# yanielc/medical-vision-textural-bias

Hardware: AMD Instinct MI355X
Metric: BraTS 4ch 240^3 vols/sec filtered+train-step @1/2/4/8 GPU; filter HBM GB/s (higher is better)
Workload: dtype f32

## Files before the change

### include/texbias.h

```cpp
#ifndef TEXBIAS_H
#define TEXBIAS_H

#include <stddef.h>
#include <stdint.h>

#ifdef __cplusplus
extern "C" {
#endif

#define TB_VERSION 1

#define TB_OK 0
#define TB_ERR_INVALID_ARG 1
#define TB_ERR_UNSUPPORTED_SIZE 2
#define TB_ERR_HIP 3
#define TB_ERR_WORKSPACE 4

#define TB_OP_NONE 0
#define TB_OP_DISK 1
#define TB_OP_GIBBS 2
#define TB_OP_LAYER 3
#define TB_OP_WRAP 4
#define TB_OP_SPIKE 5
#define TB_OP_ZF 6
// ... 104 lines not shown
int tb_channel_sum_ws_f32(const float* x, float* out, int64_t N, int64_t C, int64_t S, void* ws, size_t ws_bytes,
                          void* stream);

int tb_conv3d_small_f32(const float* x, const float* w, const float* b, float* y, int N, int Cin, int Cout, int D,
                        int H, int W, void* stream);
int tb_conv3d_small_add_f32(const float* x, const float* w, const float* b, const float* add, float* y, int N, int Cin,
                            int Cout, int D, int H, int W, void* stream);

int tb_conv3d_s2_fewin_f32(const float* in, const float* K, const float* bias, float* out, int N, int Cin, int Mout,
                           int Do, int Ho, int Wo, void* stream);
int tb_convT3d_fewout_f32(const float* x, const float* W, const float* bias, float* y, int N, int Cin, int Mout, int Di,
                          int Hi, int Wi, void* stream);
int tb_conv3d_fwd16_f32(const float* x, const float* W, const float* bias, float* y, int N, int D, int H, int Wd,
                        void* stream);
int tb_conv3d_fwd16_add_f32(const float* x, const float* W, const float* bias, const float* add, float* y, int N, int D,
                            int H, int Wd, void* stream);
int tb_conv3d_fwd16_dgrad_f32(const float* gy, const float* W, const float* add, int64_t add_sn, float* dx, int N, int D,
                              int H, int Wd, void* stream);

int tb_convT3d_mfma64_f32(const float* x, const float* W, const float* bias, float* y, int N, int Di, int Hi, int Wi,
                          void* stream);
int tb_convT3d_mfma_f32(const float* x, const float* W, const float* bias, float* y, int N, int Cin, int Di, int Hi,
                        int Wi, void* stream);

int tb_conv3d_mfma_f32(const float* x, const float* W, const float* bias, float* y, int N, int C, int D, int H, int Wd,
                       void* stream);
int tb_conv3d_mfma_add_f32(const float* x, const float* W, const float* bias, const float* add, float* y, int N, int C,
                           int D, int H, int Wd, void* stream);
int tb_conv3d_mfma_dgrad_f32(const float* gy, const float* W, const float* add, int64_t add_sn, float* dx, int N, int C,
                             int D, int H, int Wd, void* stream);

#define TB_CG_CONV 0
#define TB_CG_DGRAD 1
#define TB_CG_CONVT 2
size_t tb_conv3d_gemm_workspace_bytes(int mode, int N, int Cin, int M, int D, int H, int Wd, int stride, int ksize);
int tb_conv3d_gemm_f32(int mode, const float* x, int64_t xsn, const float* W, const float* bias, const float* add,
                       int64_t addsn, float* y, int64_t ysn, int N, int Cin, int M, int D, int H, int Wd, int stride,
                       int ksize, void* ws, size_t ws_bytes, void* stream);
int tb_conv3d_gemm_config(int mode, int N, int Cin, int M, int D, int H, int Wd, int stride, int ksize, int64_t* cfg);

size_t tb_conv3d_wgrad_gemm_ws_bytes(int N, int M, int C, int Do, int Ho, int Wo, int Di, int Hi, int Wi, int stride,
                                     int ksize);
int tb_conv3d_wgrad_gemm_f32(const float* G, int64_t gsn, const float* X, int64_t xsn, float* dW, int N, int M, int C,
                             int Do, int Ho, int Wo, int Di, int Hi, int Wi, int stride, int ksize, void* ws,
                             size_t ws_bytes, void* stream);
int tb_conv3d_wgrad_gemm_config(int N, int M, int C, int Do, int Ho, int Wo, int Di, int Hi, int Wi, int stride,
// ... 69 lines not shown
```

### medical-vision-textural-bias_amd/csrc/conv_up.hip

```cpp
#include <hip/hip_runtime.h>

#include <cstdlib>
#include <type_traits>

#include "conv_host.h"
#include "split_bf16.h"
#include "texbias.h"

namespace {

typedef float f2v __attribute__((ext_vector_type(2)));
typedef float f32x4 __attribute__((ext_vector_type(4)));
typedef const __attribute__((address_space(4))) float* cfloat_p;
typedef const __attribute__((address_space(4))) f2v* cf2v_p;

template <int B, int N, class F>
__device__ __forceinline__ void static_for(F&& f) {
  if constexpr (B < N) {
    f(std::integral_constant<int, B>{});
    static_for<B + 1, N>(f);
  }
}

struct S2Args {
// ... 811 lines not shown
#define TB_F16(X, PF)                                                                                             \
  case X:                                                                                                         \
    kern = add ? (NS == 4 ? k_conv3d_fwd16<YB, X, 512, true, PF, 4> : k_conv3d_fwd16<YB, X, 512, true, PF, 3>)     \
               : (NS == 4 ? k_conv3d_fwd16<YB, X, 512, false, PF, 4> : k_conv3d_fwd16<YB, X, 512, false, PF, 3>);  \
    break;
  switch (Wd / 16) {
    TB_F16(1, false) TB_F16(2, false) TB_F16(3, false) TB_F16(4, false) TB_F16(5, true) TB_F16(6, false)
    TB_F16(7, false) TB_F16(8, false)
    default: return TB_ERR_UNSUPPORTED_SIZE;
  }
#undef TB_F16
  a.ncol = N * a.nyb;
  unsigned nblk = (unsigned)(N * a.nyb * a.ZS);
  a.persist = per_cu == 1 && (int64_t)a.ncol * D >= 8LL * tb::num_cu() && nblk % tb::num_cu() != 0;
  if (a.persist) nblk = (unsigned)tb::num_cu();
  return tb::launch_lds(kern, dim3(nblk), dim3(512), lds, reinterpret_cast<hipStream_t>(stream), a);
}

namespace {
struct T64Args {
  const float* x;
  const float* W;
  const float* bias;
  float* y;
  int Di, Hi, Wi;
  int ZS, zlen, nyb;
  int PX, RX;
};

template <int G, int YB, int NL>
__global__ __launch_bounds__(256) void k_convT_mfma64(T64Args a) {
  extern __shared__ __attribute__((aligned(16))) float smem[];
  constexpr int NR = YB + 1;
  constexpr int CIN = 16 * G, HT = 4 / G;
  const int tid = (int)threadIdx.x, lane = tid & 63;
  const int w = __builtin_amdgcn_readfirstlane(tid >> 6);
  const int g = w % G, h = w / G;
  const int Di = a.Di, Hi = a.Hi, Wi = a.Wi, PX = a.PX, RX = a.RX, SS = CIN * RX;
  float* ring = smem;
  float* part = smem + 2 * SS;
  for (int i = tid; i < 2 * SS; i += 256) ring[i] = 0.f;
  int b = (int)blockIdx.x;
  const int zs = b % a.ZS;
  b /= a.ZS;
  const int yb = b % a.nyb, n = b / a.nyb;
  const int y0 = yb * YB;
  const int z0 = zs * a.zlen, z1 = min(Di, z0 + a.zlen);
  const int li = lane & 15, ks = lane >> 4;
  float af[108];
#pragma unroll
// ... 21 lines not shown
      const bool ok = in && gof[j] >= 0;
      rg[j] = *reinterpret_cast<const float4*>(src + gch[j] * cstride + (ok ? gof[j] : 0));
    }
  };
  auto store = [&](int zi) {
    float* d = ring + (zi & 1) * SS;
    const bool in = zi < Di;
#pragma unroll
    for (int j = 0; j < NL; ++j)
      *reinterpret_cast<float4*>(d + lof[j]) = (in && gof[j] >= 0) ? rg[j] : make_float4(0.f, 0.f, 0.f, 0.f);
  };
  float bm[4];
#pragma unroll
  for (int r = 0; r < 4; ++r) bm[r] = a.bias ? a.bias[4 * ks + r] : 0.f;
  __syncthreads();
  load(z0);
  store(z0);
  load(z0 + 1);
  store(z0 + 1);
  __builtin_amdgcn_s_waitcnt(0x0F70);
  __syncthreads();
  const int npos = YB * Wi, ntile = (npos + 15) / 16;
  const int64_t oplane = 4 * plane, orow = 2 * Wi;
  float* yb0 = a.y + (int64_t)n * 16 * (2 * Di) * oplane;
  auto sums = [&](int z, int t0, int pb) {
    const float* pr = part + pb * 4 * 8 * 256;
    for (int k = w; k < 4 * HT; k += 4) {
      const int hq = k >> 2, pz = (k >> 1) & 1, py = k & 1, q0 = pz * 4 + py * 2;
      const int pq = 16 * (t0 + hq) + li, yq = pq / Wi, xq = pq - yq * Wi;
      const bool okp = t0 + hq < ntile && pq < npos && y0 + yq < Hi;
#pragma unroll
      for (int r = 0; r < 4; ++r) {
        const int m = 4 * ks + r, e = m * 16 + li;
        float v0 = bm[r], v1 = bm[r];
#pragma unroll
        for (int v = 0; v < G; ++v) {
          v0 += pr[((hq * G + v) * 8 + q0) * 256 + e];
          v1 += pr[((hq * G + v) * 8 + q0 + 1) * 256 + e];
        }
        if (okp)
          *reinterpret_cast<float2*>(yb0 + ((int64_t)m * (2 * Di) + 2 * z + pz) * oplane +
                                     (int64_t)(2 * (y0 + yq) + py) * orow + 2 * xq) = make_float2(v0, v1);
      }
    }
  };
  int buf = 0;
  for (int z = z0; z < z1; ++z) {
    if (z + 1 < z1) load(z + 2);
    const float* sz[2] = {ring + (z & 1) * SS, ring + ((z + 1) & 1) * SS};
    for (int t0 = 0; t0 < ntile; t0 += HT) {
      const int tI = t0 + h;
      const int p = 16 * tI + li, pc = p < npos ? p : npos - 1;
      const int yy = pc / Wi, xx = pc - yy * Wi;
      const int bl = (16 * g + ks) * RX + yy * PX + xx;
      f32x4 acc[8];
#pragma unroll
      for (int q = 0; q < 8; ++q) acc[q] = f32x4{0.f, 0.f, 0.f, 0.f};
#pragma unroll
      for (int tz = 0; tz < 3; ++tz)
#pragma unroll
        for (int ty = 0; ty < 3; ++ty)
#pragma unroll
// ... 1 lines not shown
            const int t = tz * 9 + ty * 3 + tx;
            const int par = (tz != 1) * 4 + (ty != 1) * 2 + (tx != 1);
            const float* s = sz[tz == 0] + bl + (ty == 0) * PX + (tx == 0);
#pragma unroll
            for (int cq = 0; cq < 4; ++cq)
              acc[par] = __builtin_amdgcn_mfma_f32_16x16x4f32(af[4 * t + cq], s[4 * cq * RX], acc[par], 0, 0, 0);
          }
      float* pw = part + (buf * 4 + w) * 8 * 256;
#pragma unroll
      for (int q = 0; q < 8; ++q)
#pragma unroll
        for (int r = 0; r < 4; ++r) pw[q * 256 + (4 * ks + r) * 16 + li] = acc[q][r];
      __syncthreads();
      if (t0 > 0) sums(z, t0 - HT, buf ^ 1);
      buf ^= 1;
    }
    store(z + 2);
    sums(z, ((ntile - 1) / HT) * HT, buf ^ 1);
    __syncthreads();
  }
}
}

int tb_convT3d_mfma64_f32(const float* x, const float* W, const float* bias, float* y, int N, int Di, int Hi, int Wi,
                          void* stream) {
  return tb_convT3d_mfma_f32(x, W, bias, y, N, 64, Di, Hi, Wi, stream);
}

int tb_convT3d_mfma_f32(const float* x, const float* W, const float* bias, float* y, int N, int Cin, int Di, int Hi,
                        int Wi, void* stream) {
  if (!x || !W || !y || N < 1 || Di < 1 || Hi < 1 || Wi < 1) return TB_ERR_INVALID_ARG;
  if (Cin != 32 && Cin != 64) return TB_ERR_UNSUPPORTED_SIZE;
  if (Wi % 4 != 0 || Wi > 64 || (reinterpret_cast<uintptr_t>(x) & 15) != 0 || (reinterpret_cast<uintptr_t>(y) & 7) != 0)
    return TB_ERR_UNSUPPORTED_SIZE;
  constexpr int YB = 2;
  T64Args a{};
  a.x = x, a.W = W, a.bias = bias, a.y = y, a.Di = Di, a.Hi = Hi, a.Wi = Wi;
  a.PX = Wi + 4;
  a.RX = (YB + 1) * a.PX;
  while ((a.RX & 31) != 16) ++a.RX;
  a.nyb = (Hi + YB - 1) / YB;
  const size_t lds = (size_t)4 * (2 * Cin * a.RX + 2 * 4 * 8 * 256);
  if (lds > 163840) return TB_ERR_UNSUPPORTED_SIZE;
  a.zlen = tb::zseg(Di, N * a.nyb, 1, 1);
  a.ZS = (Di + a.zlen - 1) / a.zlen;
  const int nl = (Cin * (YB + 1) * (Wi / 4) + 255) / 256;
  void (*kern)(T64Args) = nullptr;
  switch (nl) {
#define TB_NL(k) \
  case k: kern = Cin == 64 ? k_convT_mfma64<4, YB, k> : k_convT_mfma64<2, YB, k>; break;
    TB_NL(1) TB_NL(2) TB_NL(3) TB_NL(4) TB_NL(5) TB_NL(6) TB_NL(7) TB_NL(8) TB_NL(9) TB_NL(10) TB_NL(11) TB_NL(12)
#undef TB_NL
    default: return TB_ERR_UNSUPPORTED_SIZE;
  }
  return tb::launch_lds(kern, dim3((unsigned)(N * a.nyb * a.ZS)), dim3(256), lds,
                        reinterpret_cast<hipStream_t>(stream), a);
}

namespace {
struct S1Args {
  const float* x;
  const float* W;
  const float* bias;
  const float* add;
  float* y;
  int D, H, Wd, YB;
  int ZS, zlen, nyb, MG;
  int PX, RX;
  int flip;
  int64_t addsn;
};

template <int G, int NC, int NL, int NTH, bool ADD = false>
__global__ __launch_bounds__(NTH) void k_conv3d_mfma_s1(S1Args a) {
  constexpr int CIN = 16 * G, MTB = 4 / G, NWG = NTH / 256;
  extern __shared__ __attribute__((aligned(16))) float smem[];
  const int tid = (int)threadIdx.x, lane = tid & 63;
  const int w = __builtin_amdgcn_readfirstlane(tid >> 6);
  const int g = w % G, mt = (w / G) % MTB, h = w / 4;
// ... 408 lines not shown
```

### medical-vision-textural-bias_amd/texbias/_lib.py

```python
from __future__ import annotations

import ctypes as C
import os
import threading

from ._abi import TB_OK

PKG_DIR = os.path.dirname(os.path.dirname(os.path.abspath(__file__)))
LIB_PATH = os.environ.get("TEXBIAS_LIB", os.path.join(PKG_DIR, "libtexbias.so"))

_lock = threading.Lock()
_lib = None


class TexbiasError(RuntimeError):
    pass


def _proto(L):
    P, I, I64, U64, F, SZ = C.c_void_p, C.c_int, C.c_int64, C.c_uint64, C.c_float, C.c_size_t
    sig = {
        "tb_version": (I, []),
        "tb_error_string": (C.c_char_p, [I]),
        "tb_last_hip_error": (I, []),
# ... 23 lines not shown
        "tb_conv3d_wgrad_bias_ws_f32": (I, [P, P, P, P] + [I] * 11 + [P, SZ, P, P]),
        "tb_instnorm_prelu_workspace_bytes": (SZ, [I64]),
        "tb_instnorm_prelu_fwd_f32": (I, [P, P, P, P, P, I64, I64, F, P, SZ, P]),
        "tb_instnorm_prelu_bwd_f32": (I, [P, P, P, P, P, P, P, I64, I64, P, SZ, P]),
        "tb_channel_sum_f32": (I, [P, P, I64, I64, I64, P]),
        "tb_channel_sum_ws_bytes": (SZ, [I64, I64, I64]),
        "tb_channel_sum_ws_f32": (I, [P, P, I64, I64, I64, P, SZ, P]),
        "tb_adn_workspace_bytes": (SZ, [I64, I64, I64]),
        "tb_adam_f32": (I, [I, P, P, P, P, P, P, P] + [C.c_double] * 5 + [I, P]),
        "tb_adn_counters": (I64, [I64, I64]),
        "tb_adn_fwd_f32": (I, [P, I64, P, I64, P, I64, P, P, P, I64, I64, I64, F, P, SZ, P, P]),
        "tb_adn_bwd_f32": (I, [P, I64, P, I64, P, I64, P, P, P, P, P, P, I64, I64, I64, P, SZ, P, P]),
        "tb_conv3d_small_f32": (I, [P, P, P, P] + [I] * 6 + [P]),
        "tb_conv3d_small_add_f32": (I, [P, P, P, P, P] + [I] * 6 + [P]),
        "tb_conv3d_fwd16_add_f32": (I, [P, P, P, P, P] + [I] * 4 + [P]),
        "tb_conv3d_mfma_add_f32": (I, [P, P, P, P, P] + [I] * 5 + [P]),
        "tb_conv3d_mfma_dgrad_f32": (I, [P, P, P, I64, P] + [I] * 5 + [P]),
        "tb_conv3d_fwd16_dgrad_f32": (I, [P, P, P, I64, P] + [I] * 4 + [P]),
        "tb_conv3d_s2_fewin_f32": (I, [P, P, P, P] + [I] * 6 + [P]),
        "tb_convT3d_fewout_f32": (I, [P, P, P, P] + [I] * 6 + [P]),
        "tb_conv3d_fwd16_f32": (I, [P, P, P, P] + [I] * 4 + [P]),
        "tb_convT3d_mfma64_f32": (I, [P, P, P, P] + [I] * 4 + [P]),
        "tb_convT3d_mfma_f32": (I, [P, P, P, P] + [I] * 5 + [P]),
        "tb_conv3d_mfma_f32": (I, [P, P, P, P] + [I] * 5 + [P]),
        "tb_conv3d_gemm_workspace_bytes": (SZ, [I] * 9),
        "tb_conv3d_gemm_f32": (I, [I, P, I64, P, P, P, I64, P, I64] + [I] * 8 + [P, SZ, P]),
        "tb_conv3d_gemm_config": (I, [I] * 9 + [P]),
        "tb_conv3d_wgrad_gemm_ws_bytes": (SZ, [I] * 11),
        "tb_conv3d_wgrad_gemm_f32": (I, [P, I64, P, I64, P] + [I] * 11 + [P, SZ, P]),
        "tb_conv3d_wgrad_gemm_config": (I, [I] * 11 + [P]),
        "tb_conv3d_wgrad_gemm_ws_bytes_ex": (SZ, [I] * 12),
        "tb_conv3d_wgrad_gemm_ex_f32": (I, [P, I64, P, I64, P] + [I] * 12 + [P, SZ, P]),
        "tb_conv3d_wgrad_gemm_config_ex": (I, [I] * 12 + [P]),
        "tb_dice_sums_f32": (I, [P, P, P, I64, I64, I, I, P]),
        "tb_dice_sums_ws_bytes": (SZ, [I64, I64]),
        "tb_dice_sums_ws_f32": (I, [P, P, P, I64, I64, I, I, P, SZ, P]),
        "tb_dice_sums_bwd_f32": (I, [P, P, P, P, I64, I64, I, I, P]),
        "tb_dice_metric_sums_f32": (I, [P, P, P, I64, I64, P]),
        "tb_dice_loss_f32": (I, [P, P, I64, I64, I, I, F, F, P]),
        "tb_dice_loss_bwd_f32": (I, [P, P, P, I64, I64, I, I, F, F, P]),
        "tb_set_compiled_plans": (I, [I]),
        "tb_set_chain_chunk": (I, [I]),
        "tb_set_pass_timing": (I, [I]),
        "tb_get_pass_times_ms": (I, [P, P]),
        "tb_get_pass_stats": (I, [P, P, P]),
        "tb_pass_kernel": (C.c_char_p, [I]),
# ... 38 lines not shown
```

### medical-vision-textural-bias_amd/texbias/conv.py

```python
from __future__ import annotations

import ctypes
import functools
import math
import os

import torch
import torch.nn as nn
import torch.nn.functional as F

from ._lib import TexbiasError, check, lib

MIN_K_PER_OUTPUT = 64
ENABLED = os.environ.get("TEXBIAS_WGRAD", "1") != "0"
CONVT64 = True
CONVMFMA = True
CONV16 = True


def _stream(t: torch.Tensor) -> int:
    return torch.cuda.current_stream(t.device).cuda_stream


@functools.lru_cache(maxsize=256)
# ... 174 lines not shown
        return False
    k, s, p = w.shape[2], stride[0], padding[0]
    if not ((k == 3 and p == 1 and s in (1, 2)) or (k == 1 and p == 0 and s == 1 and not transposed)):
        return False
    if transposed:
        if s != 2 or tuple(output_padding) != (1, 1, 1):
            return False
        g_shape = tuple(x.shape)
        x_shape = (x.shape[0], w.shape[1]) + tuple(2 * n for n in x.shape[2:])
    else:
        g_shape, x_shape = (x.shape[0], w.shape[0]) + tuple(out_spatial), tuple(x.shape)
    if not WGRAD_GEMM_MIN_POS <= math.prod(g_shape[2:]) <= WGRAD_GEMM_MAX_POS or \
            g_shape[1] * x_shape[1] < WGRAD_GEMM_MIN_MC:
        return False
    return _wgg_ws_bytes(g_shape[0], g_shape[1], x_shape[1], *g_shape[2:], *x_shape[2:], s, k, 0) > 0


GEMM = os.environ.get("TEXBIAS_CONVGEMM", "1") != "0"
GEMM_T = False
GEMM_1 = False
GEMM_TDX = False
FWD16_DX_ADD = True
MFMA_DX_ADD = False


def _gemm_geom_ok(x: torch.Tensor, w: torch.Tensor, stride, padding, transposed: bool, output_padding) -> bool:
    if not (GEMM and custom_backward_applies(x, w) and x.dim() == 5 and len(set(stride)) == 1 and
            len(set(padding)) == 1):
        return False
    k = tuple(w.shape[2:])
    s, p = stride[0], padding[0]
    if transposed:
        ok = k == (3, 3, 3) and s == 2 and p == 1 and tuple(output_padding) == (1, 1, 1) and x.shape[1] == w.shape[0]
    else:
        ok = x.shape[1] == w.shape[1] and ((k == (3, 3, 3) and p == 1 and s in (1, 2)) or
                                           (k == (1, 1, 1) and p == 0 and s == 1 and GEMM_1))
    return ok and x.shape[1] % 8 == 0 and x.numel() // x.shape[1] * 8 * max(w.shape[0], w.shape[1], x.shape[1]) < 2 ** 31


def gemm_applies(x, w, stride, padding, transposed: bool, output_padding=(0, 0, 0)) -> bool:
    return (GEMM_T or not transposed) and _gemm_geom_ok(x, w, stride, padding, transposed, output_padding)


def gemm_dgrad_applies(gy, x, w, stride, padding, transposed: bool, output_padding=(0, 0, 0)) -> bool:
    if not (_gemm_geom_ok(x, w, stride, padding, transposed, output_padding) and gy.is_cuda and
            gy.dtype == torch.float32):
# ... 66 lines not shown
                                          b.data_ptr() if b is not None else None, y.data_ptr(), N, Cin, Cout, D, H,
                                          W, _stream(x)), "tb_convT3d_fewout_f32")
    return y


def _s2_shape_ok(spatial) -> bool:
    D, H, W = spatial
    return D % 2 == 0 and H % 2 == 0 and W % 4 == 0 and W <= 160


def s2_fewin_applies(x: torch.Tensor, w: torch.Tensor, stride, padding) -> bool:
    return custom_backward_applies(x, w) and x.dim() == 5 and tuple(w.shape[2:]) == (3, 3, 3) and \
        x.shape[1] == w.shape[1] and tuple(stride) == (2, 2, 2) and tuple(padding) == (1, 1, 1) and w.shape[1] <= 4 and \
        w.shape[0] in (16, 32) and _s2_shape_ok(x.shape[2:]) and x.data_ptr() % 16 == 0


def convT_fewout_applies(x: torch.Tensor, w: torch.Tensor, stride, padding, output_padding) -> bool:
    return custom_backward_applies(x, w) and x.dim() == 5 and tuple(w.shape[2:]) == (3, 3, 3) and \
        x.shape[1] == w.shape[0] and tuple(stride) == (2, 2, 2) and tuple(padding) == (1, 1, 1) and \
        tuple(output_padding) == (1, 1, 1) and w.shape[1] <= 4 and w.shape[0] in (16, 32) and x.shape[-1] % 4 == 0 and x.shape[-1] <= 80 and \
        _s2_shape_ok(tuple(2 * n for n in x.shape[2:]))


def convT_mfma(x: torch.Tensor, w: torch.Tensor, b) -> torch.Tensor:
    x = x.contiguous()
    N, Cin, D, H, W = x.shape
    y = torch.empty((N, 16, 2 * D, 2 * H, 2 * W), dtype=torch.float32, device=x.device)
    with torch.cuda.device(x.device):
        check(lib().tb_convT3d_mfma_f32(x.data_ptr(), w.contiguous().data_ptr(),
                                        b.data_ptr() if b is not None else None, y.data_ptr(), N, Cin, D, H, W,
                                        _stream(x)), "tb_convT3d_mfma_f32")
    return y


convT_mfma64 = convT_mfma


def s2_dgrad_applies(gy: torch.Tensor, x: torch.Tensor, w: torch.Tensor, stride, padding) -> bool:
    return CONVT64 and gy.is_cuda and gy.dtype == torch.float32 and w.dtype == torch.float32 and \
        tuple(w.shape) == (32, 16, 3, 3, 3) and tuple(stride) == (2, 2, 2) and gy.shape[1] == 32 and \
        tuple(padding) == (1, 1, 1) and gy.dim() == 5 and all(2 * a == b for a, b in zip(gy.shape[2:], x.shape[2:])) and \
        gy.shape[-1] % 4 == 0 and gy.shape[-1] <= 64 and gy.data_ptr() % 16 == 0


def convT64_applies(x: torch.Tensor, w: torch.Tensor, stride, padding, output_padding) -> bool:
    return CONVT64 and custom_backward_applies(x, w) and x.dim() == 5 and tuple(w.shape) == (64, 16, 3, 3, 3) and \
        x.shape[1] == 64 and \
        tuple(stride) == (2, 2, 2) and tuple(padding) == (1, 1, 1) and tuple(output_padding) == (1, 1, 1) and \
        x.shape[-1] % 4 == 0 and x.shape[-1] <= 64 and x.data_ptr() % 16 == 0


def conv_fwd16(x: torch.Tensor, w: torch.Tensor, b, add=None) -> torch.Tensor:
    x = x.contiguous()
    N, _, D, H, W = x.shape
# ... 165 lines not shown
            if k == "small":
                return small_conv(x, w, b, add)
            return conv_gemm(x, w, b, "convT" if self.transposed else "conv", self.stride[0], self.k, add=add)
        if add is not None:
            return self.forward(x, w, b).add_(add)
        if k == "fwd16":
            return conv_fwd16(x, w, b)
        if k == "mfma":
            return conv_mfma(x, w, b)
        if k == "fewin":
            return conv_s2_fewin(x, s2_pairs(w), b, w.shape[0])
        if k == "small":
            return small_conv(x, w, b)
        if k == "fewout":
            return convT_fewout(x, w, b)
        if k == "convT64":
            return convT_mfma(x, w, b)
        if k == "gemm":
            return conv_gemm(x, w, b, "convT" if self.transposed else "conv", self.stride[0], self.k)
        if self.transposed:
            return F.conv_transpose3d(x, w, b, self.stride, self.padding, self.output_padding)
        return F.conv3d(x, w, b, self.stride, self.padding)

    def input_grad(self, gy, x, w, add=None):
        k = self.dx
        if add is not None:
            if k == "fwd16" and FWD16_DX_ADD:
                return conv_fwd16_dgrad(gy, w, add)
            if k == "mfma" and MFMA_DX_ADD:
                return conv_mfma_dgrad(gy, w, add)
            if k == "small":
                return small_conv(gy, w.flip(2, 3, 4).transpose(0, 1).contiguous(), None, add.contiguous())
            if k == "gemm" and not self.transposed and self.stride[0] == 1:
                return conv_gemm(gy, w, None, "dgrad", 1, w.shape[2], add=add.contiguous())
            return self.input_grad(gy, x, w).add_(add)
        if k == "fwd16":
            return conv_fwd16_dgrad(gy, w)
        if k == "mfma":
            return conv_mfma_dgrad(gy, w)
        if k == "small":
            return small_conv(gy, w.flip(2, 3, 4).transpose(0, 1).contiguous(), None)
        if k == "fewout":
            return conv_s2_fewin(gy, s2_pairs(w), None, w.shape[0])
        if k == "convT64":
            return convT_mfma(gy if gy.data_ptr() % 16 == 0 else gy.clone(), w, None)
        if k == "gemm":
            return gemm_dgrad(gy, w, self.stride[0], self.transposed)
        gx, _, _ = torch.ops.aten.convolution_backward(
            gy, x, w, None, list(self.stride), list(self.padding), [1, 1, 1], self.transposed,
            list(self.output_padding), 1, [True, False, False])
        return gx
# ... 72 lines not shown
```

### medical-vision-textural-bias_amd/texbias/unet.py

```python
from __future__ import annotations

import os
from typing import Sequence

import torch
import torch.nn as nn

from . import conv as _conv
from .conv import Conv3d, ConvTranspose3d
from . import norm as _norm
from .norm import adn_backward, adn_forward, instnorm_prelu

FUSED = os.environ.get("TEXBIAS_FUSED_UNITS", "1") != "0"


def _fusable(x: torch.Tensor, conv: nn.Module, adn) -> bool:
    if not (FUSED and _norm.ENABLED and x.is_cuda and x.dtype == torch.float32 and
            isinstance(conv, (Conv3d, ConvTranspose3d)) and conv.groups == 1 and conv.dilation == (1, 1, 1) and
            _conv.custom_backward_applies(x, conv.weight)):
        return False
    if isinstance(conv, Conv3d) and conv.padding_mode != "zeros":
        return False
    return adn is None or adn.D.p == 0.0 or not adn.training

# ... 41 lines not shown
        need_b = ctx.has_b and n[2]
        gb = None
        if n[1] and need_b:
            gw, gb = ctx.route.weight_bias_grad(g, x, w)
        else:
            gw = ctx.route.weight_grad(g, x, w) if n[1] else None
        if need_b and gb is None:
            gb = _conv.channel_sum(g)
        return gx, gw, gb, None


def _adjacent(a: torch.Tensor, b: torch.Tensor):
    if not (a.is_contiguous() and b.is_contiguous() and a.shape[1:] == b.shape[1:] and a.dtype == b.dtype and
            a.untyped_storage().data_ptr() == b.untyped_storage().data_ptr() and
            b.storage_offset() == a.storage_offset() + a.numel()):
        return None
    return torch.empty(0, dtype=a.dtype, device=a.device).set_(
        a.untyped_storage(), a.storage_offset(), (a.shape[0] + b.shape[0],) + tuple(a.shape[1:]))


class _StackedUnitFn(torch.autograd.Function):

    @staticmethod
    def forward(ctx, x, w0, b0, wr, br, a0w, w1, b1, a1w, unit, eps, skip):
        c = w0.shape[0]
        w_st = _adjacent(w0, wr)
        if w_st is None:
            w_st = torch.cat([w0, wr], 0)
        b_st = None
        if b0 is not None and br is not None:
            b_st = _adjacent(b0, br)
            if b_st is None:
                b_st = torch.cat([b0, br], 0)
        x = x.contiguous()
        r_st = unit.stacked_route(x, w_st)
        y2 = r_st.forward(x, w_st, b_st)
        z0, res = y2[:, :c], y2[:, c:]
        a0, m0, s0 = adn_forward(z0, a0w, eps)
        conv1 = list(unit.conv.children())[1].conv
        r1 = _conv.route_of(conv1, a0)
        z1 = r1.forward(a0, w1, b1)
        out, m1, s1 = adn_forward(z1, a1w, eps, res=res)
        ctx.save_for_backward(x, w_st, a0w, w1, a1w, y2, a0, z1, m0, s0, m1, s1)
        ctx.cfg = (c, r_st, r1, b0 is not None, b1 is not None)
        ctx.skip = skip
        return out

    @staticmethod
    def backward(ctx, g):
        x, w_st, a0w, w1, a1w, y2, a0, z1, m0, s0, m1, s1 = ctx.saved_tensors
        c, r_st, r1, has_b0, has_b1 = ctx.cfg
        n = ctx.needs_input_grad
        dy2 = torch.empty_like(y2)
        gs = ctx.skip.pop("g", None)
        if gs is not None:
            g = torch.add(g, gs, out=dy2[:, c:])
        else:
            g = g.contiguous()
            dy2[:, c:].copy_(g)
        dbr = torch.empty(c, dtype=g.dtype, device=g.device) if has_b0 and n[4] else None
        dz1, da1, db1 = adn_backward(z1, g, m1, s1, a1w, need_w=n[8], need_bias=has_b1, dysum_out=dbr)
        da0 = r1.input_grad(dz1, a0, w1)
        gw1 = r1.weight_grad(dz1, a0, w1) if n[6] else None
        _, dw0a, db0 = adn_backward(y2[:, :c], da0, m0, s0, a0w, need_w=n[5], need_bias=has_b0,
                                    dx_out=dy2[:, :c])
        gx = r_st.input_grad(dy2, x, w_st) if n[0] else None
        gw_st = r_st.weight_grad(dy2, x, w_st) if (n[1] or n[3]) else None
        return (gx, gw_st[:c] if gw_st is not None else None, db0, gw_st[c:] if gw_st is not None else None, dbr,
                dw0a, gw1, db1 if n[7] else None, da1, None, None, None)


class ADN(nn.Sequential):
    def __init__(self, channels: int, dropout: float = 0.0):
        super().__init__()
        self.add_module("N", nn.InstanceNorm3d(channels, eps=1e-5, affine=False, track_running_stats=False))
        self.add_module("D", nn.Dropout(p=dropout))
        self.add_module("A", nn.PReLU(num_parameters=1))

    def forward(self, x):
        if _norm.ENABLED and x.is_cuda and x.dtype == torch.float32 and (self.D.p == 0.0 or not self.training):
            return instnorm_prelu(x, self.A.weight, self.N.eps)
        return super().forward(x)


class Convolution(nn.Sequential):
    def __init__(self, cin: int, cout: int, strides: int = 1, kernel_size: int = 3, conv_only: bool = False,
                 is_transposed: bool = False, dropout: float = 0.0):
        super().__init__()
        pad = (kernel_size - 1) // 2
        if is_transposed:
            conv = ConvTranspose3d(cin, cout, kernel_size, stride=strides, padding=pad, output_padding=strides - 1)
        else:
# ... 33 lines not shown
            self.residual = nn.Identity()
        self._register_state_dict_hook(ResidualUnit._unshare_packed)

    @staticmethod
    def _unshare_packed(module, state_dict, prefix, local_metadata):
        for k in ("conv.unit0.conv.weight", "conv.unit0.conv.bias", "residual.weight", "residual.bias"):
            v = state_dict.get(prefix + k)
            if v is not None and not isinstance(v, nn.Parameter) and v.untyped_storage().nbytes() != \
                    v.numel() * v.element_size():
                state_dict[prefix + k] = v.clone()
        return state_dict

    def forward(self, x):
        units = list(self.conv.children())
        if isinstance(self.residual, Conv3d) and len(units) == 2 and all(hasattr(u, "adn") for u in units):
            u0, u1 = units
            r = self.residual
            if r.stride == u0.conv.stride and r.kernel_size == u0.conv.kernel_size and r.padding == u0.conv.padding \
                    and isinstance(u0.conv, Conv3d) and _fusable(x, u0.conv, u0.adn) and _fusable(x, r, None) and \
                    _fusable(x, u1.conv, u1.adn) and (r.bias is None) == (u0.conv.bias is None) and \
                    u0.adn.N.eps == u1.adn.N.eps and r.padding_mode == "zeros":
                skip = {}
                y = _StackedUnitFn.apply(x, u0.conv.weight, u0.conv.bias, r.weight, r.bias, u0.adn.A.weight,
                                         u1.conv.weight, u1.conv.bias, u1.adn.A.weight, self, u0.adn.N.eps, skip)
                y._tb_skip = skip
                return y
        if isinstance(self.residual, nn.Identity) and len(units) == 1 and hasattr(units[0], "adn"):
            out = self.__dict__.pop("_tb_out", None)
            if out is not None and tuple(out.shape) != tuple(x.shape[:1]) + (units[0].conv.out_channels,) + \
                    tuple(x.shape[2:]):
                out = None
            y = units[0].fused(x, res=x, out=out)
            if y is not None:
                return y
        if isinstance(self.residual, nn.Identity) and len(units) == 1 and not hasattr(units[0], "adn") and \
                _fusable(x, units[0].conv, None):
            c = units[0].conv
            return _ConvResFn.apply(x, c.weight, c.bias, _conv.route_of(c, x))
        res = self.residual(x)
        return self.conv(x) + res

    def pack_parameters(self) -> bool:
        units = list(self.conv.children())
        if not (isinstance(self.residual, Conv3d) and len(units) == 2 and hasattr(units[0], "conv")):
            return False
        c0, r = units[0].conv, self.residual
        if torch.is_inference_mode_enabled() or not isinstance(c0, Conv3d) or r.stride != c0.stride or \
# ... 122 lines not shown
```

Baseline: 197.4.

## Fuse skip-gradient add into transposed-conv dgrad and add split-bf16 convT kernel

Adds an add/strided-output variant of the transposed-conv MFMA kernel so the backward pass of a stacked residual unit can accumulate the upstream skip gradient and write directly into the concatenated dy2 buffer of the next unit. This is meant to remove a separate elementwise add and a copy into the concat buffer. It also adds a new 512-thread split-bf16 (3-way) MFMA kernel for Cin=64 with parity-class tap decomposition, plus a YB=1 fallback for larger widths. The cost is more complex autograd bookkeeping through shared skip dicts, and numerical differences from the bf16 split path.

After: 201.7, median of 6. +2.2%, better.

```diff
diff --git a/include/texbias.h b/include/texbias.h
--- a/include/texbias.h
+++ b/include/texbias.h
@@ -150,6 +150,8 @@
                           void* stream);
 int tb_convT3d_mfma_f32(const float* x, const float* W, const float* bias, float* y, int N, int Cin, int Di, int Hi,
                         int Wi, void* stream);
+int tb_convT3d_mfma_add_f32(const float* x, const float* W, const float* bias, const float* add, int64_t add_sn,
+                            float* y, int64_t y_sn, int N, int Cin, int Di, int Hi, int Wi, void* stream);
 
 int tb_conv3d_mfma_f32(const float* x, const float* W, const float* bias, float* y, int N, int C, int D, int H, int Wd,
                        void* stream);
diff --git a/medical-vision-textural-bias_amd/csrc/conv_up.hip b/medical-vision-textural-bias_amd/csrc/conv_up.hip
--- a/medical-vision-textural-bias_amd/csrc/conv_up.hip
+++ b/medical-vision-textural-bias_amd/csrc/conv_up.hip
@@ -857,10 +857,12 @@
   const float* x;
   const float* W;
   const float* bias;
+  const float* add;
   float* y;
   int Di, Hi, Wi;
   int ZS, zlen, nyb;
   int PX, RX;
+  int64_t ysn, addsn;
 };
 
 template <int G, int YB, int NL>
@@ -928,13 +930,22 @@
   __syncthreads();
   const int npos = YB * Wi, ntile = (npos + 15) / 16;
   const int64_t oplane = 4 * plane, orow = 2 * Wi;
-  float* yb0 = a.y + (int64_t)n * 16 * (2 * Di) * oplane;
+  float* yb0 = a.y + (int64_t)n * a.ysn;
+  const float* ab0 = a.add ? a.add + (int64_t)n * a.addsn : nullptr;
   auto sums = [&](int z, int t0, int pb) {
     const float* pr = part + pb * 4 * 8 * 256;
     for (int k = w; k < 4 * HT; k += 4) {
       const int hq = k >> 2, pz = (k >> 1) & 1, py = k & 1, q0 = pz * 4 + py * 2;
       const int pq = 16 * (t0 + hq) + li, yq = pq / Wi, xq = pq - yq * Wi;
       const bool okp = t0 + hq < ntile && pq < npos && y0 + yq < Hi;
+      float2 av[4];
+      if (ab0) {
+#pragma unroll
+        for (int r = 0; r < 4; ++r)
+          av[r] = okp ? *reinterpret_cast<const float2*>(ab0 + ((int64_t)(4 * ks + r) * (2 * Di) + 2 * z + pz) * oplane +
+                                                         (int64_t)(2 * (y0 + yq) + py) * orow + 2 * xq)
+                      : make_float2(0.f, 0.f);
+      }
 #pragma unroll
       for (int r = 0; r < 4; ++r) {
         const int m = 4 * ks + r, e = m * 16 + li;
@@ -944,6 +955,7 @@
           v0 += pr[((hq * G + v) * 8 + q0) * 256 + e];
           v1 += pr[((hq * G + v) * 8 + q0 + 1) * 256 + e];
         }
+        if (ab0) v0 += av[r].x, v1 += av[r].y;
         if (okp)
           *reinterpret_cast<float2*>(yb0 + ((int64_t)m * (2 * Di) + 2 * z + pz) * oplane +
                                      (int64_t)(2 * (y0 + yq) + py) * orow + 2 * xq) = make_float2(v0, v1);
@@ -991,39 +1003,286 @@
 }
 }
 
+namespace {
+struct TSArgs {
+  const float* x;
+  const float* W;
+  const float* bias;
+  const float* add;
+  float* y;
+  int Di, Hi, Wi, YB;
+  int ZS, zlen, nyb;
+  int ntile;
+  int64_t ysn, addsn;
+};
+
+struct CtTap {
+  int t, dz, dy, dx;
+};
+constexpr CtTap ct_tap(int cls, int j) {
+  const int pz = (cls >> 2) & 1, py = (cls >> 1) & 1, px = cls & 1;
+  const int nx = 1 + px, ny = 1 + py;
+  const int ix = j % nx, iy = (j / nx) % ny, iz = j / (nx * ny);
+  return CtTap{(pz ? (iz ? 0 : 2) : 1) * 9 + (py ? (iy ? 0 : 2) : 1) * 3 + (px ? (ix ? 0 : 2) : 1), pz ? iz : 0,
+               py ? iy : 0, px ? ix : 0};
+}
+constexpr int ct_ntap(int cls) { return (1 + ((cls >> 2) & 1)) * (1 + ((cls >> 1) & 1)) * (1 + (cls & 1)); }
+constexpr int ct_cls(int half, int s) {
+  return half == 0 ? (s < 4 ? 7 : s < 6 ? 3 : 0) : (s < 2 ? 5 : s < 4 ? 6 : s == 4 ? 1 : s == 5 ? 2 : 4);
+}
+constexpr int ct_pair(int half, int s) { return half == 0 ? (s < 4 ? s : s < 6 ? s - 4 : 0) : (s < 4 ? (s & 1) : 0); }
+constexpr CtTap ct_step_tap(int half, int s, int hi) {
+  const int cls = ct_cls(half, s), e = 2 * ct_pair(half, s) + hi;
+  return ct_tap(cls, e < ct_ntap(cls) ? e : ct_ntap(cls) - 1);
+}
+constexpr bool ct_step_pad(int half, int s, int hi) { return 2 * ct_pair(half, s) + hi >= ct_ntap(ct_cls(half, s)); }
+
+template <int HALF>
+__device__ __forceinline__ void ct_mma(const tb::bf16x8 (&af)[7][3], const char* rb, int sb0, int sb1, int RPB, int SPL,
+                                       int hv, char* pw) {
+  using tb::bf16x8;
+  bf16x8 bq[2][3];
+  auto ldb = [&](int s, bf16x8 (&bf)[3]) {
+    const CtTap t0 = ct_step_tap(HALF, s, 0), t1 = ct_step_tap(HALF, s, 1);
+    const int c0 = (t0.dz ? sb1 : sb0) + t0.dy * RPB + t0.dx * 32;
+    const int c1 = (t1.dz ? sb1 : sb0) + t1.dy * RPB + t1.dx * 32;
+    const int o = hv ? c1 : c0;
+    bf[1] = *reinterpret_cast<const bf16x8*>(rb + o + SPL);
+    bf[2] = *reinterpret_cast<const bf16x8*>(rb + o + 2 * SPL);
+    bf[0] = *reinterpret_cast<const bf16x8*>(rb + o);
+  };
+  tb::f32x4s c = {0.f, 0.f, 0.f, 0.f}, cs = c;
+  ldb(0, bq[0]);
+#pragma unroll
+  for (int s = 0; s < 7; ++s) {
+    if (s + 1 < 7) ldb(s + 1, bq[(s + 1) & 1]);
+    tb::mfma_split6(af[s], bq[s & 1], c, cs);
+    if (s == 6 || ct_cls(HALF, s + 1) != ct_cls(HALF, s)) {
+      c += cs;
+      *reinterpret_cast<tb::f32x4s*>(pw + ct_cls(HALF, s) * 1024) = c;
+      c = tb::f32x4s{0.f, 0.f, 0.f, 0.f}, cs = c;
+    }
+  }
+  __builtin_amdgcn_sched_group_barrier(0x100, 3, 0);
+#pragma unroll
+  for (int s = 0; s < 6; ++s) {
+    __builtin_amdgcn_sched_group_barrier(0x100, 3, 0);
+    __builtin_amdgcn_sched_group_barrier(0x008, 6, 0);
+  }
+  __builtin_amdgcn_sched_group_barrier(0x008, 6, 0);
+}
+
+template <bool ADD>
+__global__ __launch_bounds__(512) void k_convT_split(TSArgs a) {
+  using tb::bf16x8;
+  constexpr int G = 4, NTH = 512;
+  extern __shared__ __attribute__((aligned(16))) char ringt[];
+  const int tid = (int)threadIdx.x, lane = tid & 63;
+  const int w = __builtin_amdgcn_readfirstlane(tid >> 6);
+  const int grp = w & 3, half = w >> 2;
+  const int Di = a.Di, Hi = a.Hi, Wi = a.Wi, YB = a.YB, NR = YB + 1;
+  const int RPB = (Wi + 1) * 32, GPB = NR * RPB, SPL = G * GPB, SLOT = 3 * SPL;
+  char* part = ringt + 2 * SLOT;
+  for (int i = tid; i < 2 * SLOT / 16; i += NTH) reinterpret_cast<uint4*>(ringt)[i] = make_uint4(0, 0, 0, 0);
+  int b = (int)blockIdx.x;
+  const int zs = b % a.ZS;
+  b /= a.ZS;
+  const int yb = b % a.nyb, n = b / a.nyb;
+  const int y0 = yb * YB;
+  const int z0 = zs * a.zlen, z1 = min(Di, z0 + a.zlen);
+  const int li = lane & 15, g4 = lane >> 4, hi = g4 >> 1;
+  bf16x8 af[7][3];
+  {
+    const float* wl = a.W + ((16 * grp + 8 * (g4 & 1)) * 16 + li) * 27;
+#pragma unroll
+    for (int s = 0; s < 7; ++s) {
+      const int t = half ? (hi ? ct_step_tap(1, s, 1).t : ct_step_tap(1, s, 0).t)
+                         : (hi ? ct_step_tap(0, s, 1).t : ct_step_tap(0, s, 0).t);
+      const bool pad = hi && (half ? ct_step_pad(1, s, 1) : ct_step_pad(0, s, 1));
+      float v[8];
+#pragma unroll
+      for (int j = 0; j < 8; ++j) v[j] = wl[j * 16 * 27 + t];
+#pragma unroll
+      for (int j = 0; j < 8; ++j) v[j] = pad ? 0.f : v[j];
+      tb::split3(v, af[s][0], af[s][1], af[s][2]);
+    }
+  }
+  const int64_t plane = (int64_t)Hi * Wi, cstride = (int64_t)Di * plane;
+  const char* xb = reinterpret_cast<const char*>(a.x + (int64_t)n * 16 * G * cstride);
+  const int W4 = Wi >> 2, ntask = 4 * NR * W4 * G;
+  const int tk = tid < ntask ? tid : tid % ntask;
+  const int cq = tk & 3, rr = (tk >> 2) % NR, r2 = (tk >> 2) / NR, q4 = r2 % W4, sg = r2 / W4;
+  const int lof = sg * GPB + rr * RPB + 4 * q4 * 32 + cq * 8;
+  const int yi = y0 + rr;
+  const bool rowok = yi < Hi;
+  const unsigned chb = (unsigned)(4 * cstride);
+  const unsigned gof = rowok ? (unsigned)(16 * sg + 4 * cq) * chb + 4u * (unsigned)(yi * Wi + 4 * q4) : 0u;
+  float4 rg[4];
+  auto load = [&](int zi) {
+    const char* src = xb + (int64_t)(zi >= Di ? Di - 1 : zi) * plane * 4;
+#pragma unroll
+    for (int c = 0; c < 4; ++c) rg[c] = *reinterpret_cast<const float4*>(src + c * chb + gof);
+  };
+  auto store = [&](int zi) {
+    char* d = ringt + (zi & 1) * SLOT + lof;
+    const unsigned m = 0u - (unsigned)(rowok && zi < Di);
+#pragma unroll
+    for (int e = 0; e < 4; ++e) {
+      float v[4];
+#pragma unroll
+      for (int c = 0; c < 4; ++c)
+        v[c] = __uint_as_float(__float_as_uint(e == 0 ? rg[c].x : e == 1 ? rg[c].y : e == 2 ? rg[c].z : rg[c].w) & m);
+      unsigned p[3][2];
+      tb::split3_pk(v[0], v[1], p[0][0], p[1][0], p[2][0]);
+      tb::split3_pk(v[2], v[3], p[0][1], p[1][1], p[2][1]);
+#pragma unroll
+      for (int s = 0; s < 3; ++s) *reinterpret_cast<uint2*>(d + s * SPL + e * 32) = make_uint2(p[s][0], p[s][1]);
+    }
+  };
+  const int pzs = (w >> 1) & 1, pys = w & 1, q0 = pzs * 4 + pys * 2, rh = w >> 2;
+  const int m0 = 4 * g4 + 2 * rh;
+  const float bm[2] = {a.bias ? a.bias[m0] : 0.f, a.bias ? a.bias[m0 + 1] : 0.f};
+  __syncthreads();
+  load(z0);
+  store(z0);
+  load(z0 + 1);
+  store(z0 + 1);
+  __builtin_amdgcn_s_waitcnt(0x0F70);
+  __syncthreads();
+  const int npos = YB * Wi, ntile = a.ntile;
+  const int64_t oplane = 4 * plane, orow = 2 * Wi, och = 2 * Di * oplane;
+  float* yb0 = a.y + (int64_t)n * a.ysn;
+  const float* ab0 = ADD ? a.add + (int64_t)n * a.addsn : nullptr;
+  const int lb = grp * GPB + 16 * (g4 & 1);
+  int buf = 0;
+  for (int z = z0; z < z1; ++z) {
+    load(z + 2);
+    int hv = hi;
+    asm volatile("" : "+v"(hv));
+    const int sb0 = (z & 1) * SLOT, sb1 = ((z + 1) & 1) * SLOT;
+    auto tile = [&](int t, auto LAST) {
+      const int p = 16 * t + li, pc = p < npos ? p : npos - 1;
+      const int yy = pc / Wi, xx = pc - yy * Wi;
+      const bool ok = p < npos && y0 + yy < Hi;
+      const int64_t oo = ((int64_t)m0 * (2 * Di) + 2 * z + pzs) * oplane +
+                         (int64_t)(2 * min(y0 + yy, Hi - 1) + pys) * orow + 2 * xx;
+      float2 av[2];
+      if constexpr (ADD) {
+#pragma unroll
+        for (int r = 0; r < 2; ++r) av[r] = *reinterpret_cast<const float2*>(ab0 + oo + r * och);
+      }
+      const char* rb = ringt + lb + yy * RPB + xx * 32;
+      char* pw = part + (buf * 4 + grp) * 8192 + lane * 16;
+      if (half == 0)
+        ct_mma<0>(af, rb, sb0, sb1, RPB, SPL, hv, pw);
+      else
+        ct_mma<1>(af, rb, sb0, sb1, RPB, SPL, hv, pw);
+      __syncthreads();
+      if constexpr (decltype(LAST)::value) store(z + 2);
+      const char* pr = part + (buf * 32 + q0) * 1024 + lane * 16 + 8 * rh;
+      tb::f32x2s v0 = *reinterpret_cast<const tb::f32x2s*>(pr), v1 = *reinterpret_cast<const tb::f32x2s*>(pr + 1024);
+#pragma unroll
+      for (int gg = 1; gg < G; ++gg) {
+        v0 += *reinterpret_cast<const tb::f32x2s*>(pr + gg * 8192);
+        v1 += *reinterpret_cast<const tb::f32x2s*>(pr + gg * 8192 + 1024);
+      }
+#pragma unroll
+      for (int r = 0; r < 2; ++r) {
+        float2 o = make_float2(v0[r] + bm[r], v1[r] + bm[r]);
+        if constexpr (ADD) o.x += av[r].x, o.y += av[r].y;
+        if (ok) *reinterpret_cast<float2*>(yb0 + oo + r * och) = o;
+      }
+      buf ^= 1;
+    };
+    for (int t = 0; t + 1 < ntile; ++t) tile(t, std::false_type{});
+    tile(ntile - 1, std::true_type{});
+    __syncthreads();
+  }
+}
+}
+
 int tb_convT3d_mfma64_f32(const float* x, const float* W, const float* bias, float* y, int N, int Di, int Hi, int Wi,
                           void* stream) {
   return tb_convT3d_mfma_f32(x, W, bias, y, N, 64, Di, Hi, Wi, stream);
 }
 
-int tb_convT3d_mfma_f32(const float* x, const float* W, const float* bias, float* y, int N, int Cin, int Di, int Hi,
-                        int Wi, void* stream) {
+static bool ct_plan(int Cin, int Di, int Hi, int Wi, TSArgs& s, size_t& lds) {
+  if (Cin != 64 || Wi < 32 || (int64_t)Cin * Di * Hi * Wi >= (1LL << 29)) return false;
+  for (int YB = std::min(2, Hi); YB >= 1; --YB) {
+    lds = (size_t)2 * 3 * 4 * (YB + 1) * (Wi + 1) * 32 + 65536;
+    if (4 * 4 * (YB + 1) * (Wi / 4) > 512 || lds > 163840) continue;
+    s.Di = Di, s.Hi = Hi, s.Wi = Wi, s.YB = YB;
+    s.ntile = (YB * Wi + 15) / 16;
+    s.nyb = (Hi + YB - 1) / YB;
+    return true;
+  }
+  return false;
+}
+
+static int convT_call(const float* x, const float* W, const float* bias, const float* add, int64_t add_sn, float* y,
+                      int64_t y_sn, int N, int Cin, int Di, int Hi, int Wi, void* stream) {
   if (!x || !W || !y || N < 1 || Di < 1 || Hi < 1 || Wi < 1) return TB_ERR_INVALID_ARG;
   if (Cin != 32 && Cin != 64) return TB_ERR_UNSUPPORTED_SIZE;
   if (Wi % 4 != 0 || Wi > 64 || (reinterpret_cast<uintptr_t>(x) & 15) != 0 || (reinterpret_cast<uintptr_t>(y) & 7) != 0)
     return TB_ERR_UNSUPPORTED_SIZE;
-  constexpr int YB = 2;
+  const int64_t ysz = (int64_t)16 * 8 * Di * Hi * Wi;
+  if (y_sn == 0) y_sn = ysz;
+  if (add_sn == 0) add_sn = ysz;
+  if (y_sn < ysz || (y_sn & 1) != 0 || (add && (add_sn < ysz || (add_sn & 1) != 0 || (reinterpret_cast<uintptr_t>(add) & 7) != 0)))
+    return TB_ERR_UNSUPPORTED_SIZE;
+  hipStream_t st = reinterpret_cast<hipStream_t>(stream);
+  {
+    TSArgs s{};
+    size_t slds = 0;
+    if (ct_plan(Cin, Di, Hi, Wi, s, slds)) {
+      s.x = x, s.W = W, s.bias = bias, s.add = add, s.y = y, s.ysn = y_sn, s.addsn = add_sn;
+      s.zlen = tb::zseg(Di, N * s.nyb, 1, 1);
+      s.ZS = (Di + s.zlen - 1) / s.zlen;
+      return tb::launch_lds(add ? k_convT_split<true> : k_convT_split<false>, dim3((unsigned)(N * s.nyb * s.ZS)),
+                            dim3(512), slds, st, s);
+    }
+  }
   T64Args a{};
-  a.x = x, a.W = W, a.bias = bias, a.y = y, a.Di = Di, a.Hi = Hi, a.Wi = Wi;
+  a.x = x, a.W = W, a.bias = bias, a.add = add, a.y = y, a.Di = Di, a.Hi = Hi, a.Wi = Wi;
+  a.ysn = y_sn, a.addsn = add_sn;
   a.PX = Wi + 4;
-  a.RX = (YB + 1) * a.PX;
-  while ((a.RX & 31) != 16) ++a.RX;
+  int YB = 2;
+  size_t lds = 0;
+  for (; YB >= 1; --YB) {
+    a.RX = (YB + 1) * a.PX;
+    while ((a.RX & 31) != 16) ++a.RX;
+    lds = (size_t)4 * (2 * Cin * a.RX + 2 * 4 * 8 * 256);
+    if (lds <= 163840) break;
+  }
+  if (YB < 1) return TB_ERR_UNSUPPORTED_SIZE;
   a.nyb = (Hi + YB - 1) / YB;
-  const size_t lds = (size_t)4 * (2 * Cin * a.RX + 2 * 4 * 8 * 256);
-  if (lds > 163840) return TB_ERR_UNSUPPORTED_SIZE;
   a.zlen = tb::zseg(Di, N * a.nyb, 1, 1);
   a.ZS = (Di + a.zlen - 1) / a.zlen;
   const int nl = (Cin * (YB + 1) * (Wi / 4) + 255) / 256;
   void (*kern)(T64Args) = nullptr;
-  switch (nl) {
+  if (YB == 1) {
+    if (Cin == 64 && nl == 8) kern = k_convT_mfma64<4, 1, 8>;
+  } else {
+    switch (nl) {
 #define TB_NL(k) \
-  case k: kern = Cin == 64 ? k_convT_mfma64<4, YB, k> : k_convT_mfma64<2, YB, k>; break;
-    TB_NL(1) TB_NL(2) TB_NL(3) TB_NL(4) TB_NL(5) TB_NL(6) TB_NL(7) TB_NL(8) TB_NL(9) TB_NL(10) TB_NL(11) TB_NL(12)
+  case k: kern = Cin == 64 ? k_convT_mfma64<4, 2, k> : k_convT_mfma64<2, 2, k>; break;
+      TB_NL(1) TB_NL(2) TB_NL(3) TB_NL(4) TB_NL(5) TB_NL(6) TB_NL(7) TB_NL(8) TB_NL(9) TB_NL(10) TB_NL(11) TB_NL(12)
 #undef TB_NL
-    default: return TB_ERR_UNSUPPORTED_SIZE;
-  }
-  return tb::launch_lds(kern, dim3((unsigned)(N * a.nyb * a.ZS)), dim3(256), lds,
-                        reinterpret_cast<hipStream_t>(stream), a);
+      default: break;
+    }
+  }
+  if (!kern) return TB_ERR_UNSUPPORTED_SIZE;
+  return tb::launch_lds(kern, dim3((unsigned)(N * a.nyb * a.ZS)), dim3(256), lds, st, a);
+}
+
+int tb_convT3d_mfma_f32(const float* x, const float* W, const float* bias, float* y, int N, int Cin, int Di, int Hi,
+                        int Wi, void* stream) {
+  return convT_call(x, W, bias, nullptr, 0, y, 0, N, Cin, Di, Hi, Wi, stream);
+}
+
+int tb_convT3d_mfma_add_f32(const float* x, const float* W, const float* bias, const float* add, int64_t add_sn,
+                            float* y, int64_t y_sn, int N, int Cin, int Di, int Hi, int Wi, void* stream) {
+  return convT_call(x, W, bias, add, add_sn, y, y_sn, N, Cin, Di, Hi, Wi, stream);
 }
 
 namespace {
diff --git a/medical-vision-textural-bias_amd/texbias/_lib.py b/medical-vision-textural-bias_amd/texbias/_lib.py
--- a/medical-vision-textural-bias_amd/texbias/_lib.py
+++ b/medical-vision-textural-bias_amd/texbias/_lib.py
@@ -69,6 +69,7 @@
         "tb_conv3d_fwd16_f32": (I, [P, P, P, P] + [I] * 4 + [P]),
         "tb_convT3d_mfma64_f32": (I, [P, P, P, P] + [I] * 4 + [P]),
         "tb_convT3d_mfma_f32": (I, [P, P, P, P] + [I] * 5 + [P]),
+        "tb_convT3d_mfma_add_f32": (I, [P, P, P, P, I64, P, I64] + [I] * 5 + [P]),
         "tb_conv3d_mfma_f32": (I, [P, P, P, P] + [I] * 5 + [P]),
         "tb_conv3d_gemm_workspace_bytes": (SZ, [I] * 9),
         "tb_conv3d_gemm_f32": (I, [I, P, I64, P, P, P, I64, P, I64] + [I] * 8 + [P, SZ, P]),
diff --git a/medical-vision-textural-bias_amd/texbias/conv.py b/medical-vision-textural-bias_amd/texbias/conv.py
--- a/medical-vision-textural-bias_amd/texbias/conv.py
+++ b/medical-vision-textural-bias_amd/texbias/conv.py
@@ -220,6 +220,7 @@
 GEMM_TDX = False
 FWD16_DX_ADD = True
 MFMA_DX_ADD = False
+CONVT_DX_ADD = True
 
 
 def _gemm_geom_ok(x: torch.Tensor, w: torch.Tensor, stride, padding, transposed: bool, output_padding) -> bool:
@@ -332,14 +333,37 @@
         _s2_shape_ok(tuple(2 * n for n in x.shape[2:]))
 
 
-def convT_mfma(x: torch.Tensor, w: torch.Tensor, b) -> torch.Tensor:
+def _sample_stride(t: torch.Tensor, shape) -> int:
+    if tuple(t.shape) != tuple(shape) or t.dtype != torch.float32 or not t[0].is_contiguous():
+        return -1
+    return t.stride(0)
+
+
+def convT_mfma(x: torch.Tensor, w: torch.Tensor, b, add=None, out=None) -> torch.Tensor:
     x = x.contiguous()
     N, Cin, D, H, W = x.shape
-    y = torch.empty((N, 16, 2 * D, 2 * H, 2 * W), dtype=torch.float32, device=x.device)
+    shape = (N, 16, 2 * D, 2 * H, 2 * W)
+    if add is None and out is None:
+        y = torch.empty(shape, dtype=torch.float32, device=x.device)
+        with torch.cuda.device(x.device):
+            check(lib().tb_convT3d_mfma_f32(x.data_ptr(), w.contiguous().data_ptr(),
+                                            b.data_ptr() if b is not None else None, y.data_ptr(), N, Cin, D, H, W,
+                                            _stream(x)), "tb_convT3d_mfma_f32")
+        return y
+    y = out if out is not None else torch.empty(shape, dtype=torch.float32, device=x.device)
+    ysn = _sample_stride(y, shape)
+    assert ysn > 0 and ysn % 2 == 0 and y.data_ptr() % 8 == 0, "out: the output's shape, samples contiguous"
+    asn = 0
+    if add is not None:
+        asn = _sample_stride(add, shape)
+        if asn <= 0 or asn % 2 or add.data_ptr() % 8:
+            add = add.contiguous()
+            asn = add.stride(0)
     with torch.cuda.device(x.device):
-        check(lib().tb_convT3d_mfma_f32(x.data_ptr(), w.contiguous().data_ptr(),
-                                        b.data_ptr() if b is not None else None, y.data_ptr(), N, Cin, D, H, W,
-                                        _stream(x)), "tb_convT3d_mfma_f32")
+        check(lib().tb_convT3d_mfma_add_f32(x.data_ptr(), w.contiguous().data_ptr(),
+                                            b.data_ptr() if b is not None else None,
+                                            add.data_ptr() if add is not None else None, asn, y.data_ptr(), ysn,
+                                            N, Cin, D, H, W, _stream(x)), "tb_convT3d_mfma_add_f32")
     return y
 
 
@@ -551,11 +575,16 @@
             return F.conv_transpose3d(x, w, b, self.stride, self.padding, self.output_padding)
         return F.conv3d(x, w, b, self.stride, self.padding)
 
-    def input_grad(self, gy, x, w, add=None):
+    def input_grad(self, gy, x, w, add=None, out=None):
         k = self.dx
+        if out is not None:
+            assert k == "convT64"
+            return convT_mfma(gy if gy.data_ptr() % 16 == 0 else gy.clone(), w, None, add=add, out=out)
         if add is not None:
             if k == "fwd16" and FWD16_DX_ADD:
                 return conv_fwd16_dgrad(gy, w, add)
+            if k == "convT64" and CONVT_DX_ADD:
+                return convT_mfma(gy if gy.data_ptr() % 16 == 0 else gy.clone(), w, None, add=add)
             if k == "mfma" and MFMA_DX_ADD:
                 return conv_mfma_dgrad(gy, w, add)
             if k == "small":
diff --git a/medical-vision-textural-bias_amd/texbias/unet.py b/medical-vision-textural-bias_amd/texbias/unet.py
--- a/medical-vision-textural-bias_amd/texbias/unet.py
+++ b/medical-vision-textural-bias_amd/texbias/unet.py
@@ -87,7 +87,7 @@
 class _StackedUnitFn(torch.autograd.Function):
 
     @staticmethod
-    def forward(ctx, x, w0, b0, wr, br, a0w, w1, b1, a1w, unit, eps, skip):
+    def forward(ctx, x, w0, b0, wr, br, a0w, w1, b1, a1w, unit, eps, skip, skip_in=None):
         c = w0.shape[0]
         w_st = _adjacent(w0, wr)
         if w_st is None:
@@ -109,6 +109,7 @@
         ctx.save_for_backward(x, w_st, a0w, w1, a1w, y2, a0, z1, m0, s0, m1, s1)
         ctx.cfg = (c, r_st, r1, b0 is not None, b1 is not None)
         ctx.skip = skip
+        ctx.skip_in = skip_in
         return out
 
     @staticmethod
@@ -116,11 +117,17 @@
         x, w_st, a0w, w1, a1w, y2, a0, z1, m0, s0, m1, s1 = ctx.saved_tensors
         c, r_st, r1, has_b0, has_b1 = ctx.cfg
         n = ctx.needs_input_grad
-        dy2 = torch.empty_like(y2)
+        dy2, gd = ctx.skip.pop("dy2", None), ctx.skip.pop("gx", None)
         gs = ctx.skip.pop("g", None)
-        if gs is not None:
+        if dy2 is not None and gd is not None and gs is None and dy2.shape == y2.shape and \
+                g.data_ptr() == gd.data_ptr() and \
+                g.shape == gd.shape and g.stride() == gd.stride():
+            pass
+        elif gs is not None:
+            dy2 = torch.empty_like(y2)
             g = torch.add(g, gs, out=dy2[:, c:])
         else:
+            dy2 = torch.empty_like(y2)
             g = g.contiguous()
             dy2[:, c:].copy_(g)
         dbr = torch.empty(c, dtype=g.dtype, device=g.device) if has_b0 and n[4] else None
@@ -129,10 +136,20 @@
         gw1 = r1.weight_grad(dz1, a0, w1) if n[6] else None
         _, dw0a, db0 = adn_backward(y2[:, :c], da0, m0, s0, a0w, need_w=n[5], need_bias=has_b0,
                                     dx_out=dy2[:, :c])
-        gx = r_st.input_grad(dy2, x, w_st) if n[0] else None
+        up = ctx.skip_in
+        gu = up.get("g") if up is not None else None
+        if n[0] and gu is not None and _conv.CONVT_DX_ADD and r_st.dx == "convT64" and gu.shape == x.shape:
+            cu = x.shape[1]
+            buf = torch.empty((x.shape[0], 2 * cu) + tuple(x.shape[2:]), dtype=x.dtype, device=x.device)
+            gx = _alias(buf, cu, 2 * cu)
+            r_st.input_grad(dy2, x, w_st, add=gu, out=gx)
+            del up["g"]
+            up["dy2"], up["gx"] = buf, gx
+        else:
+            gx = r_st.input_grad(dy2, x, w_st) if n[0] else None
         gw_st = r_st.weight_grad(dy2, x, w_st) if (n[1] or n[3]) else None
         return (gx, gw_st[:c] if gw_st is not None else None, db0, gw_st[c:] if gw_st is not None else None, dbr,
-                dw0a, gw1, db1 if n[7] else None, da1, None, None, None)
+                dw0a, gw1, db1 if n[7] else None, da1, None, None, None, None)
 
 
 class ADN(nn.Sequential):
@@ -212,7 +229,8 @@
                     u0.adn.N.eps == u1.adn.N.eps and r.padding_mode == "zeros":
                 skip = {}
                 y = _StackedUnitFn.apply(x, u0.conv.weight, u0.conv.bias, r.weight, r.bias, u0.adn.A.weight,
-                                         u1.conv.weight, u1.conv.bias, u1.adn.A.weight, self, u0.adn.N.eps, skip)
+                                         u1.conv.weight, u1.conv.bias, u1.adn.A.weight, self, u0.adn.N.eps, skip,
+                                         getattr(x, "_tb_skip", None))
                 y._tb_skip = skip
                 return y
         if isinstance(self.residual, nn.Identity) and len(units) == 1 and hasattr(units[0], "adn"):
```
